# Hi-PACE/hipace

Measured on AMD Instinct MI355X. Metric: transverse slices/s at 1024^2 x 4ppc (explicit solver), higher is better.
Workload: dtype f64

## Files before the change

### hipace_amd/api.py

```python
import ctypes as C

import numpy as np
import torch

from . import _lib
from ._lib import CIDX, COMPS, ID_VALID, PL_REAL, check


def _stream():
    return C.c_void_p(torch.cuda.current_stream().cuda_stream)


def _iarr(vals):
    return (C.c_int * len(vals))(*[int(v) for v in vals])


class Geometry:

    def __init__(self, nx, ny, lo, hi, dz, bc=1, normalized=True, consts=(1., 1., 1., 1., 1.), ng=None):
        self.nx, self.ny = nx, ny
        g = _lib.Geom()
        g.dx = (hi[0] - lo[0]) / nx
        g.dy = (hi[1] - lo[1]) / ny
        g.dz = dz
        g.xoff = 0.5 * (lo[0] + hi[0] - g.dx * (nx - 1))
        g.yoff = 0.5 * (lo[1] + hi[1] - g.dy * (ny - 1))
        g.c, g.ep0, g.mu0, g.q_e, g.m_e = consts
        g.plo = (C.c_double * 2)(lo[0], lo[1])
        g.phi = (C.c_double * 2)(hi[0], hi[1])
        g.bc = bc
        g.normalized = int(normalized)
        self.c = g


class Fields:

    def __init__(self, nx, ny, ng, ncomp, device="cuda", data=None):
        self.nx, self.ny, self.ng, self.ncomp = nx, ny, ng, ncomp
        shape = (ncomp, ny + 2 * ng, nx + 2 * ng)
        if data is None:
            self.t = torch.zeros(shape, dtype=torch.float64, device=device)
        else:
            self.t = torch.as_tensor(np.ascontiguousarray(data), dtype=torch.float64).reshape(shape).to(device).contiguous()

    def struct(self):
        s = _lib.Slab()
        s.p = self.t.data_ptr()
        s.nx, s.ny, s.ng, s.ncomp = self.nx, self.ny, self.ng, self.ncomp
        s.jstride = self.nx + 2 * self.ng
        s.nstride = s.jstride * (self.ny + 2 * self.ng)
        return s

    def numpy(self):
        return self.t.cpu().numpy()


class PlasmaSheet:

    def __init__(self, real, valid=None, ion_lev=None, device="cuda", key=None):
        real = np.ascontiguousarray(real, dtype=np.float64)
        assert real.shape[0] == 11
        self.n = real.shape[1]
        self.real = torch.as_tensor(real).to(device).contiguous()
        if valid is None:
            valid = np.ones(self.n, dtype=np.int32)
        idcpu = np.where(np.asarray(valid) != 0, np.uint64(ID_VALID | (1 << 24)), np.uint64(1 << 24)).astype(np.uint64)
        if key is not None:
            ids = (np.asarray(key, dtype=np.uint64) + np.uint64(1)) << np.uint64(24)
            idcpu = (idcpu & np.uint64(ID_VALID)) | ids
        self.idcpu = torch.as_tensor(idcpu.view(np.int64)).to(device).contiguous()
        if ion_lev is None:
            ion_lev = np.zeros(self.n, dtype=np.int32)
        self.ion_lev = torch.as_tensor(np.asarray(ion_lev, dtype=np.int32)).to(device).contiguous()

    def struct(self):
        p = _lib.Plasma()
        base = self.real.data_ptr()
        for k, name in enumerate(PL_REAL):
            setattr(p, name, base + 8 * k * self.n)
        p.idcpu = self.idcpu.data_ptr()
        p.ion_lev = self.ion_lev.data_ptr()
        p.n = self.n
        return p

    def numpy(self):
        idc = self.idcpu.cpu().numpy().view(np.uint64)
        return self.real.cpu().numpy(), ((idc >> np.uint64(63)) & np.uint64(1)).astype(np.int32)


class BoxSorter:

    def sortParticlesByBox(self, z, plo_z, dz, num_boxes):
        z = z.contiguous()
        n = z.numel()
        counts = torch.zeros(num_boxes + 1, dtype=torch.int64, device=z.device)
        offsets = torch.zeros(num_boxes + 1, dtype=torch.int64, device=z.device)
        perm = torch.zeros(max(n, 1), dtype=torch.int64, device=z.device)
        check(_lib.lib().hps_beam_sort_by_box(C.c_void_p(z.data_ptr() if n else 0), n, float(plo_z), float(dz), num_boxes,
                                              C.c_void_p(counts.data_ptr()), C.c_void_p(offsets.data_ptr()),
                                              C.c_void_p(perm.data_ptr()), _stream()))
        torch.cuda.synchronize()
        self.boxCounts = counts.cpu().numpy().astype(np.uint64)
        self.boxOffsets = offsets.cpu().numpy().astype(np.uint64)
        self.boxPermutations = perm[:n].cpu().numpy().astype(np.uint64)
        return self


class Tiling:

    def __init__(self, nx, ny, tile_size, max_particles):
        self._h = C.c_void_p()
        check(_lib.lib().hps_tiling_create(nx, ny, tile_size, max_particles, C.byref(self._h)))
        self.fallback = torch.zeros(1, dtype=torch.int32, device="cuda")

    def reorder(self, plasma, geom):
        out = PlasmaSheet.__new__(PlasmaSheet)
        out.n = plasma.n
        out.real = torch.empty_like(plasma.real)
        out.idcpu = torch.empty_like(plasma.idcpu)
        out.ion_lev = torch.empty_like(plasma.ion_lev)
        check(_lib.lib().hps_reorder_particles(self._h, plasma.struct(), out.struct(), geom.c, _stream()))
        return out

    def set_validity(self, by_weight=False, by_psi_half=False):
        check(_lib.lib().hps_tiling_set_validity(self._h, int(by_weight), int(by_psi_half)))

    def info(self):
        nt, off, perm = C.c_int(), C.c_void_p(), C.c_void_p()
        check(_lib.lib().hps_tiling_info(self._h, C.byref(nt), C.byref(off), C.byref(perm)))
        return nt.value, off.value, perm.value

    def offsets_and_perm(self, n):
        torch.cuda.synchronize()
        nt, off, perm = self.info()
        o = np.empty(nt + 2, dtype=np.int32)
        p = np.empty(n, dtype=np.uint32)
        check(_lib.lib().hps_memcpy_d2h(o.ctypes.data_as(C.c_void_p), C.c_void_p(off), o.nbytes))
        if n:
            check(_lib.lib().hps_memcpy_d2h(p.ctypes.data_as(C.c_void_p), C.c_void_p(perm), p.nbytes))
        return o, p

    def __del__(self):
        if getattr(self, "_h", None) and _lib is not None:
            _lib.lib().hps_tiling_destroy(self._h)
            self._h = None


def DepositCurrent(plasma, fields, geom, charge, mass, depos_order, jx=-1, jy=-1, jz=-1, rho=-1, chi=-1,
                   rhomjz=-1, max_qsa_weighting_factor=35.0, can_ionize=False, n_qsa=None, tiling=None, aabs=-1):
    comp = _iarr([jx, jy, jz, rho, chi, rhomjz])
    nq = C.c_void_p(n_qsa.data_ptr()) if n_qsa is not None else None
    if tiling is None:
        check(_lib.lib().hps_deposit_current_laser(fields.struct(), plasma.struct(), geom.c, comp, aabs, charge, mass,
                                                   depos_order, max_qsa_weighting_factor, int(can_ionize), nq, _stream()))
    else:
        check(_lib.lib().hps_deposit_current_tiled_laser(fields.struct(), plasma.struct(), geom.c, comp, aabs, charge, mass,
                                                         depos_order, max_qsa_weighting_factor, int(can_ionize), nq,
                                                         tiling._h, C.c_void_p(tiling.fallback.data_ptr()), _stream()))


def ExplicitDeposition(plasma, fields, geom, charge, mass, depos_order, Bz, Ez, ExmBy, EypBx, Sy, Sx,
                       derivative_type=2, can_ionize=False, tiling=None, aabs=-1):
    if tiling is None:
        check(_lib.lib().hps_explicit_deposit_laser(fields.struct(), plasma.struct(), geom.c, _iarr([Bz, Ez, ExmBy, EypBx]),
                                                    aabs, _iarr([Sy, Sx]), charge, mass, depos_order, derivative_type,
                                                    int(can_ionize), _stream()))
    else:
        check(_lib.lib().hps_explicit_deposit_tiled_laser(fields.struct(), plasma.struct(), geom.c,
                                                          _iarr([Bz, Ez, ExmBy, EypBx]), aabs, _iarr([Sy, Sx]), charge, mass,
                                                          depos_order, derivative_type, int(can_ionize), tiling._h,
                                                          C.c_void_p(tiling.fallback.data_ptr()), _stream()))


def AdvancePlasmaParticles(plasma, fields, geom, charge, mass, depos_order, Psi, Ez, Bx, By, Bz,
                           temp_slice=False, n_subcycles=1, can_ionize=False, tiling=None, aabs=-1):
    if tiling is None:
        check(_lib.lib().hps_advance_plasma_laser(fields.struct(), plasma.struct(), geom.c, _iarr([Psi, Ez, Bx, By, Bz]),
                                                  aabs, charge, mass, depos_order, int(temp_slice), n_subcycles,
                                                  int(can_ionize), _stream()))
    else:
        check(_lib.lib().hps_advance_plasma_tiled_laser(fields.struct(), plasma.struct(), geom.c,
                                                        _iarr([Psi, Ez, Bx, By, Bz]), aabs, charge, mass, depos_order,
                                                        int(temp_slice), n_subcycles, int(can_ionize), tiling._h,
                                                        C.c_void_p(tiling.fallback.data_ptr()), _stream()))


def CoulombCollision(plasma_a, plasma_b, geom, charge_a, mass_a, charge_b=None, mass_b=None, can_ionize_a=False,
                     can_ionize_b=False, coulomb_log=-1.0, background_density_SI=0.0, seed=0, collision=0, step=0, islice=0,
                     tiling_a=None, tiling_b=None):
    if plasma_b is plasma_a or charge_b is None:
        charge_b, mass_b, can_ionize_b = charge_a, mass_a, can_ionize_a
    pairs, over = C.c_long(), C.c_long()
    check(_lib.lib().hps_collide_plasma(plasma_a.struct(), tiling_a._h if tiling_a is not None else None,
                                        plasma_b.struct(), tiling_b._h if tiling_b is not None else None, geom.c, geom.nx, geom.ny,
                                        charge_a, mass_a, int(can_ionize_a), charge_b, mass_b, int(can_ionize_b), coulomb_log,
                                        background_density_SI, seed, collision, step, islice, C.byref(pairs), C.byref(over),
                                        _stream()))
    return pairs.value, over.value


class BeamSlice:

    def __init__(self, soa, nsub=None, device="cuda"):
        soa = np.ascontiguousarray(soa, dtype=np.float64)
        assert soa.ndim == 2 and soa.shape[0] == 7
        self.n = soa.shape[1]
        self.soa = torch.as_tensor(soa).to(device).contiguous()
        self.nsub = None if nsub is None else torch.as_tensor(np.ascontiguousarray(nsub, dtype=np.int32)).to(device).contiguous()
        assert self.nsub is None or self.nsub.numel() == self.n

    def struct(self):
        b = _lib.BeamSlice()
        base = self.soa.data_ptr()
        for k, name in enumerate(("x", "y", "z", "ux", "uy", "uz", "w")):
            setattr(b, name, base + 8 * k * self.n)
        b.nsub = self.nsub.data_ptr() if self.nsub is not None else None
        b.n = self.n
        return b

    def numpy(self):
        return self.soa.cpu().numpy()


def BeamPlasmaCollision(beam, plasma, geom, charge_beam, mass_beam, charge_plasma, mass_plasma, dt, can_ionize_plasma=False,
                        coulomb_log=-1.0, background_density_SI=0.0, seed=0, collision=0, step=0, islice=0):
    pairs, over = C.c_long(), C.c_long()
    check(_lib.lib().hps_collide_beam_plasma(beam.struct(), plasma.struct(), geom.c, geom.nx, geom.ny, charge_beam, mass_beam,
                                             charge_plasma, mass_plasma, int(can_ionize_plasma), coulomb_log, background_density_SI,
                                             seed, collision, step, islice, dt, C.byref(pairs), C.byref(over), _stream()))
    return pairs.value, over.value


def record_particle_dispatch(on=True):
    check(_lib.lib().hps_particles_record(int(on)))


def recorded_particle_dispatch():
    n = C.c_long()
    check(_lib.lib().hps_particles_recorded(None, 0, C.byref(n)))
    buf = C.create_string_buffer(n.value + 1)
    check(_lib.lib().hps_particles_recorded(buf, n.value + 1, C.byref(n)))
    return set(buf.value.decode().split())


class FFTPoissonSolver:

    def __init__(self, nx, ny, dx, dy, device="cuda"):
        self.nx, self.ny = nx, ny
        self._h = C.c_void_p()
        check(_lib.lib().hps_poisson_create(nx, ny, dx, dy, C.byref(self._h)))
        self.staging = torch.zeros((ny, nx), dtype=torch.float64, device=device)

    def StagingArea(self):
        return self.staging

    BACKENDS = ("own-sym", "own-pow2", "dense", "rocfft")

    def info(self):
        b, n, m = C.c_int(), C.c_int(), C.c_int()
        check(_lib.lib().hps_poisson_info(self._h, C.byref(b), C.byref(n), C.byref(m)))
        return self.BACKENDS[b.value], n.value, m.value

    def SolvePoissonEquation(self, lhs_fields, comp):
        check(_lib.lib().hps_poisson_solve(self._h, C.c_void_p(self.staging.data_ptr()), lhs_fields.struct(), comp,
                                           _stream()))

    def __del__(self):
        if getattr(self, "_h", None) and _lib is not None:
            _lib.lib().hps_poisson_destroy(self._h)
            self._h = None


class MultiGrid2:

    def __init__(self, nx, ny, dx, dy):
        self._h = C.c_void_p()
        check(_lib.lib().hps_mg2_create(nx, ny, dx, dy, C.byref(self._h)))

    def solve2(self, sol2, rhs2, acoef_real, acoef_imag, tol_rel=1e-4, tol_abs=0.0, nummaxiter=200):
        it = C.c_int()
        rn = C.c_double()
        for t in (sol2, rhs2, acoef_real, acoef_imag):
            assert t.is_cuda and t.is_contiguous() and t.dtype == torch.float64
        check(_lib.lib().hps_mg2_solve2(self._h, sol2.data_ptr(), rhs2.data_ptr(), acoef_real.data_ptr(), acoef_imag.data_ptr(),
                                        tol_rel, tol_abs, nummaxiter, C.byref(it), C.byref(rn), _stream()))
        return it.value, rn.value

    BOTTOMS = ("lower-v", "single-block", "per-sweep")
    TILES = ("single-block", "32x16", "64x32")

    def info(self):
        nl, top, b, t = C.c_int(), C.c_int(), C.c_int(), (C.c_int * 31)()
        check(_lib.lib().hps_mg2_info(self._h, C.byref(nl), C.byref(top), C.byref(b), t))
        return {"nlev": nl.value, "low_top": top.value, "bottom": self.BOTTOMS[b.value],
                "tiles": tuple(self.TILES[v] for v in t if v >= 0)}

    def __del__(self):
        if getattr(self, "_h", None) and _lib is not None:
            _lib.lib().hps_mg2_destroy(self._h)
            self._h = None


class MultiGrid:

    def __init__(self, nx, ny, dx, dy):
        self._h = C.c_void_p()
        check(_lib.lib().hps_mg_create(nx, ny, dx, dy, C.byref(self._h)))

    LOWV = ("v3", "v-cc", "v-nodal", "bottom")
    TILES = ("TileSmall", "TileBig", "TileSmall-pull", "TileMid-pull")

    def info(self):
        cc, nl, lb, kind, npyr, nres, pull1 = (C.c_int() for _ in range(7))
        lds, t = C.c_long(), (C.c_int * 31)()
        check(_lib.lib().hps_mg_info(self._h, C.byref(cc), C.byref(nl), C.byref(lb), C.byref(kind), C.byref(lds), t,
                                     C.byref(pull1), C.byref(npyr), C.byref(nres)))
        return {"cc": bool(cc.value), "nlev": nl.value, "lowv_begin": lb.value, "lowv": self.LOWV[kind.value],
                "lowv_lds": lds.value, "tiles": tuple(self.TILES[v] for v in t if v >= 0), "nodal_pull1": bool(pull1.value),
                "pyramid": npyr.value, "restricts": nres.value}

    def solve1(self, fields, sol_comp, rhs_comp, acoef_comp, tol_rel=1e-4, tol_abs=2.2250738585072014e-308,
               nummaxiter=200):
        it = C.c_int()
        rn = C.c_double()
        check(_lib.lib().hps_mg_solve1(self._h, fields.struct(), sol_comp, rhs_comp, acoef_comp, tol_rel, tol_abs,
                                       nummaxiter, C.byref(it), C.byref(rn), _stream()))
        return it.value, rn.value

    def solve1_fabs(self, sol, rhs, acoef, tol_rel=1e-4, tol_abs=2.2250738585072014e-308, nummaxiter=200):
        it = C.c_int()
        rn = C.c_double()
        check(_lib.lib().hps_mg_solve1_fabs(self._h, sol.struct(), rhs.struct(), acoef.struct(), tol_rel, tol_abs, nummaxiter,
                                            C.byref(it), C.byref(rn), _stream()))
        return it.value, rn.value

    def __del__(self):
        if getattr(self, "_h", None) and _lib is not None:
            _lib.lib().hps_mg_destroy(self._h)
            self._h = None


class AdaptiveTimeStep:

    def __init__(self, deck, density_profile=None):
        self.deck = dict(deck)
        self._dk = _lib.fill_struct(_lib.Deck(), deck)
        self._h = C.c_void_p()
        check(_lib.lib().hps_adaptive_create(C.byref(self._dk), C.byref(self._h)))
        if density_profile is not None:
            self.set_density_profile(*density_profile)

    @classmethod
    def for_engine(cls, engine):
        return cls(engine.deck, getattr(engine, "density_profile", None))

    def __del__(self):
        if getattr(self, "_h", None) and _lib is not None:
            _lib.lib().hps_adaptive_destroy(self._h)
            self._h = None

    def set_density_profile(self, r=(), fr=(), ct=(), ft=()):
        a = [np.ascontiguousarray(v, dtype=np.float64) for v in (r, fr, ct, ft)]
        assert len(a[0]) == len(a[1]) and len(a[2]) == len(a[3])
        p = [x.ctypes.data_as(C.c_void_p) if len(x) else None for x in a]
        check(_lib.lib().hps_adaptive_set_density_profile(self._h, len(a[0]), p[0], p[1], len(a[2]), p[2], p[3]))

    def initial_dt(self, uz_mean=None, uz_std=None, nstages=1):
        um = self.deck["beam_umean"][2] if uz_mean is None else uz_mean
        us = self.deck.get("beam_uz_std", 0.0) if uz_std is None else uz_std
        dt = C.c_double()
        check(_lib.lib().hps_adaptive_initial_dt(self._h, float(um), float(us), int(nstages), C.byref(dt)))
        return dt.value

    def CalculateFromDensity(self, t):
        dt = C.c_double()
        check(_lib.lib().hps_adaptive_before_step(self._h, float(t), C.byref(dt)))
        return dt.value

    def next_time(self):
        t = C.c_double()
        check(_lib.lib().hps_adaptive_next_time(self._h, C.byref(t)))
        return t.value

    def CalculateFromMinUz(self, moments, t, nstages=1):
        m = np.ascontiguousarray(moments, dtype=np.float64)
        assert m.shape == (4,)
        dt = C.c_double()
        check(_lib.lib().hps_adaptive_after_step(self._h, m.ctypes.data_as(C.c_void_p), float(t), int(nstages), C.byref(dt)))
        return dt.value


class SliceEngine:

    def __init__(self, deck, device=0, tile_size=None, sort_period=None):
        self.deck = dict(deck)
        self.step_times = []
        self._dk = _lib.fill_struct(_lib.Deck(), deck)
        self._h = C.c_void_p()
        check(_lib.lib().hps_engine_create(C.byref(self._dk), device, C.byref(self._h)))
        if tile_size is not None:
            check(_lib.lib().hps_engine_set_tiling(self._h, tile_size, sort_period or 128))
        for a, b, coulomb_log, seed in deck.get("collisions", ()):
            if a == "beam":
                self.add_beam_collision(b, coulomb_log, seed)
            else:
                self.add_collision(a, b, coulomb_log, seed)
        nc, ng, npart = C.c_int(), C.c_int(), C.c_long()
        check(_lib.lib().hps_engine_info(self._h, C.byref(nc), C.byref(ng), C.byref(npart)))
        self.ncomp, self.ng, self.nparticles = nc.value, ng.value, npart.value

    def __del__(self):
        if getattr(self, "_h", None) and _lib is not None:
            _lib.lib().hps_engine_destroy(self._h)
            self._h = None

    def begin_step(self):
        check(_lib.lib().hps_engine_begin_step(self._h))

    def solve_slice(self, islice):
        check(_lib.lib().hps_engine_solve_slice(self._h, islice))

    def solve_slice_begin(self, islice):
        check(_lib.lib().hps_engine_solve_slice_begin(self._h, islice))

    def solve_slice_finish(self, islice):
        check(_lib.lib().hps_engine_solve_slice_finish(self._h, islice))

    def slice_ready(self):
        return bool(_lib.lib().hps_engine_slice_ready(self._h))

    def run_step(self):
        check(_lib.lib().hps_engine_run_step(self._h))

    def sync(self):
        check(_lib.lib().hps_engine_sync(self._h))

    def set_tiling(self, tile_size=16, sort_period=128):
        check(_lib.lib().hps_engine_set_tiling(self._h, tile_size, sort_period))

    def add_collision(self, species_a=0, species_b=0, coulomb_log=-1.0, seed=0):
        check(_lib.lib().hps_engine_add_collision(self._h, species_a, species_b, coulomb_log, seed))

    def add_beam_collision(self, plasma_species=0, coulomb_log=-1.0, seed=0):
        check(_lib.lib().hps_engine_add_beam_collision(self._h, plasma_species, coulomb_log, seed))

    def collision_stats(self):
        a, b = C.c_long(), C.c_long()
        check(_lib.lib().hps_engine_collision_stats(self._h, C.byref(a), C.byref(b)))
        return dict(pairs_collided=a.value, overfull_cells=b.value)

    @property
    def moving(self):
        return float(self.deck.get("dt", 0.0)) != 0.0 or self.adaptive

    @property
    def adaptive(self):
        return bool(self.deck.get("dt_adaptive", 0))

    def set_time(self, t, dt):
        check(_lib.lib().hps_engine_set_time(self._h, float(t), float(dt)))

    def beam_moments(self):
        out = np.zeros(4, dtype=np.float64)
        check(_lib.lib().hps_engine_beam_moments(self._h, out.ctypes.data_as(C.c_void_p)))
        return out

    def run_adaptive(self, n_steps=None, controller=None, on_step_end=None):
        assert self.adaptive, "run_adaptive needs a deck with dt_adaptive"
        n = self.deck["n_steps"] if n_steps is None else int(n_steps)
        ats = controller or AdaptiveTimeStep.for_engine(self)
        ats.initial_dt(nstages=1)
        t, log = 0.0, []
        for step in range(n):
            if t == float("inf"):
                break
            dt = ats.CalculateFromDensity(t)
            log.append((step, t, dt))
            self.set_time(t, dt)
            self.run_step()
            ats.CalculateFromMinUz(self.beam_moments(), t, 1)
            if on_step_end is not None:
                on_step_end(step, t, dt)
            t = ats.next_time()
        return log

    def beam_capacity(self):
        n = C.c_long()
        check(_lib.lib().hps_engine_beam_capacity(self._h, C.byref(n)))
        return n.value

    def set_beam_capacity(self, cap):
        check(_lib.lib().hps_engine_set_beam_capacity(self._h, int(cap)))

    def beam_message_doubles(self):
        r = C.c_int()
        check(_lib.lib().hps_engine_beam_message_rows(self._h, C.byref(r)))
        return 1 + r.value * self.beam_capacity()

    def beam_spin(self):
        nbeam, _ = self.beam_layout()
        out = np.zeros((3, max(nbeam, 1)), dtype=np.float64)
        check(_lib.lib().hps_engine_beam_spin(self._h, out.ctypes.data_as(C.c_void_p) if nbeam else None))
        return out[:, :nbeam]

    def set_beam_import(self, on):
        check(_lib.lib().hps_engine_set_beam_import(self._h, int(on)))

    def export_beam_slice(self, islice, msg):
        check(_lib.lib().hps_engine_export_beam_slice(self._h, islice, C.c_void_p(msg.data_ptr())))

    def import_beam_slice(self, islice, msg):
        check(_lib.lib().hps_engine_import_beam_slice(self._h, islice, C.c_void_p(msg.data_ptr())))

    def beam_state(self):
        nbeam, _ = self.beam_layout()
        nz = self.deck["nz"]
        bnd = np.zeros(nz + 1, dtype=np.int64)
        soa = np.zeros((7, max(nbeam, 1)), dtype=np.float64)
        check(_lib.lib().hps_engine_beam_state(self._h, bnd.ctypes.data_as(C.c_void_p), soa.ctypes.data_as(C.c_void_p) if nbeam else None))
        return bnd, soa[:, :nbeam].reshape(7, nbeam) if nbeam else soa[:, :0]

    def set_density_profile(self, r=(), fr=(), ct=(), ft=()):
        self.density_profile = (r, fr, ct, ft)
        a = [np.ascontiguousarray(v, dtype=np.float64) for v in (r, fr, ct, ft)]
        assert len(a[0]) == len(a[1]) and len(a[2]) == len(a[3])
        p = [x.ctypes.data_as(C.c_void_p) if len(x) else None for x in a]
        check(_lib.lib().hps_engine_set_density_profile(self._h, len(a[0]), p[0], p[1], len(a[2]), p[2], p[3]))

    def set_fusion(self, on=True):
        check(_lib.lib().hps_engine_set_fusion(self._h, int(on)))

    def fallbacks(self):
        n = C.c_long()
        check(_lib.lib().hps_engine_fallbacks(self._h, C.byref(n)))
        return n.value

    def sorts(self):
        n = C.c_long()
        check(_lib.lib().hps_engine_sorts(self._h, C.byref(n)))
        return n.value

    def set_diagnostics(self, on=True):
        check(_lib.lib().hps_engine_set_diagnostics(self._h, int(on)))

    def set_profiling(self, on=True, stride=1, light=False):
        check(_lib.lib().hps_engine_set_profiling_stride(self._h, int(stride)))
        check(_lib.lib().hps_engine_set_profiling(self._h, (2 if light else 1) if on else 0))

    def beam_layout(self):
        nb = C.c_long()
        off = (C.c_long * (self.deck["nz"] + 1))()
        check(_lib.lib().hps_engine_beam_info(self._h, C.byref(nb), off))
        return nb.value, np.array(off[:], dtype=np.int64)

    def set_beam_particles(self, soa, allow_outside=False):
        soa = np.ascontiguousarray(soa, dtype=np.float64)
        assert soa.ndim == 2 and soa.shape[0] == 7
        out = C.c_long(0)
        check(_lib.lib().hps_engine_set_beam_particles(self._h, soa.shape[1], soa.ctypes.data_as(C.c_void_p),
                                                       C.byref(out) if allow_outside else None))
        return out.value

    def set_beam_storage(self, tensor, injected_beam_support=False):
        check(_lib.lib().hps_engine_set_beam_storage(self._h, C.c_void_p(tensor.data_ptr()) if tensor is not None else None))
        if tensor is not None and injected_beam_support:
            check(_lib.lib().hps_engine_assume_initial_beam_support(self._h))

    def initial_beam_into(self, tensor):
        check(_lib.lib().hps_engine_initial_beam(self._h, C.c_void_p(tensor.data_ptr())))

    def set_field_diagnostic(self, names, coarsening=(1, 1, 1), diag_type="xyz", patch_lo=None, patch_hi=None):
        idx = _lib.CIDX_PC if self.deck.get("bxby_solver", 0) else _lib.CIDX
        cn = self.comp_names()
        comps = (C.c_int * len(names))(*[idx[n] if n in idx else cn.index(n) for n in names])
        co = (C.c_int * 3)(*coarsening)
        sd = {"xyz": -1, "yz": 0, "xz": 1, "xy": 2}[diag_type]
        plo = (C.c_double * 3)(*patch_lo) if patch_lo is not None else None
        phi = (C.c_double * 3)(*patch_hi) if patch_hi is not None else None
        check(_lib.lib().hps_engine_set_field_diagnostic_box(self._h, len(names), comps, co, sd, plo, phi))
        self._fd = (list(names), tuple(coarsening))

    def field_diagnostic_geometry(self):
        n, lo, hi = (C.c_int * 3)(), (C.c_double * 3)(), (C.c_double * 3)()
        check(_lib.lib().hps_engine_field_diagnostic_geometry(self._h, n, lo, hi))
        return tuple(n), tuple(lo), tuple(hi)

    def field_diagnostic(self):
        names, _ = self._fd
        n, _, _ = self.field_diagnostic_geometry()
        out = np.empty((len(names), n[2], n[1], n[0]))
        check(_lib.lib().hps_engine_field_diagnostic(self._h, out.ctypes.data_as(C.c_void_p)))
        return {k: out[i] for i, k in enumerate(names)}

    INSITU_FIELDS = ["[Ex^2]", "[Ey^2]", "[Ez^2]", "[Bx^2]", "[By^2]", "[Bz^2]", "[ExmBy^2]", "[EypBx^2]", "[jz_beam]",
                     "[Ez*jz_beam]"]

    INSITU_PLASMA = ["sum(w)", "[x]", "[x^2]", "[y]", "[y^2]", "[ux]", "[ux^2]", "[uy]", "[uy^2]", "[uz]", "[uz^2]", "[ga]",
                     "[ga^2]", "[(ga-1)*(1-vz)]", "Np"]

    INSITU_BEAM = ["sum(w)", "[x]", "[x^2]", "[y]", "[y^2]", "[z]", "[z^2]", "[ux]", "[ux^2]", "[uy]", "[uy^2]", "[uz]", "[uz^2]",
                   "[x*ux]", "[y*uy]", "[z*uz]", "[x*uy]", "[y*ux]", "[ux/uz]", "[uy/uz]", "[ga]", "[ga^2]", "Np"]

    def laser_vcycles(self):
        n = C.c_long()
        check(_lib.lib().hps_engine_laser_vcycles(self._h, C.byref(n)))
        return n.value

    def set_insitu_beam(self, radius=float("inf")):
        check(_lib.lib().hps_engine_set_insitu_beam(self._h, min(float(radius), 1.0e300)))

    def insitu_beam(self):
        out = np.empty((23, self.deck["nz"]))
        check(_lib.lib().hps_engine_insitu_beam(self._h, out.ctypes.data_as(C.c_void_p)))
        return {n: out[i] for i, n in enumerate(self.INSITU_BEAM)}

    def set_insitu_plasma(self, radius=float("inf")):
        check(_lib.lib().hps_engine_set_insitu_plasma(self._h, min(float(radius), 1.0e300)))

    def insitu_plasma(self):
        out = np.empty((15, self.deck["nz"]))
        check(_lib.lib().hps_engine_insitu_plasma(self._h, out.ctypes.data_as(C.c_void_p)))
        return {n: out[i] for i, n in enumerate(self.INSITU_PLASMA)}

    def set_insitu_fields(self, on=True):
        check(_lib.lib().hps_engine_set_insitu_fields(self._h, int(on)))

    def insitu_fields(self):
        out = np.empty((10, self.deck["nz"]))
        check(_lib.lib().hps_engine_insitu_fields(self._h, out.ctypes.data_as(C.c_void_p)))
        return {n: out[i] for i, n in enumerate(self.INSITU_FIELDS)}

    def stream_handle(self):
        return _lib.lib().hps_engine_stream(self._h)

    def record_event(self, slot):
        ev = C.c_void_p()
        check(_lib.lib().hps_engine_record_event(self._h, int(slot), C.byref(ev)))
        return ev.value

    def wait_event(self, event):
        if event is not None:
            check(_lib.lib().hps_engine_wait_event(self._h, C.c_void_p(event)))

    def copy_async(self, dst, src):
        assert dst.numel() == src.numel()
        check(_lib.lib().hps_engine_copy_async(self._h, C.c_void_p(dst.data_ptr()), C.c_void_p(src.data_ptr()),
                                               dst.numel() * 8))

    def phase_times(self):
        ms = (C.c_double * 8)()
        n = C.c_long()
        check(_lib.lib().hps_engine_phase_times(self._h, ms, C.byref(n)))
        names = ["deposit_current", "poisson", "explicit_deposit", "mg_solve1", "advance_plasma", "other", "sort", "empty_interval"]
        return {k: ms[i] for i, k in enumerate(names)}, n.value

    def checksums(self):
        out = (C.c_double * self.ncomp)()
        check(_lib.lib().hps_engine_checksums(self._h, out))
        names = self.comp_names()
        cs = {names[i]: out[i] for i in range(self.ncomp)}
        if "aabs" in cs:
            tot = C.c_double()
            check(_lib.lib().hps_engine_laser_info(self._h, None, C.byref(tot)))
            cs["laserEnvelope"] = tot.value
        return cs

    @property
    def has_laser(self):
        return bool(self.deck.get("laser_on", 0))

    def laser_message_doubles(self):
        return 4 * self.deck["nx"] * self.deck["ny"]

    def set_step(self, step):
        check(_lib.lib().hps_engine_set_step(self._h, int(step)))

    def set_laser_import(self, on, step=0):
        check(_lib.lib().hps_engine_set_laser_import(self._h, int(on), int(step)))

    def export_laser_slice(self, islice, msg):
        check(_lib.lib().hps_engine_export_laser_slice(self._h, islice, C.c_void_p(msg.data_ptr())))

    def import_laser_slice(self, islice, msg):
        check(_lib.lib().hps_engine_import_laser_slice(self._h, islice, C.c_void_p(msg.data_ptr())))

    def import_laser_from(self, islice, src):
        check(_lib.lib().hps_engine_import_laser_from(self._h, islice, src._h))

    def laser_envelope(self):
        d = self.deck
        out = np.empty((d["nz"], d["ny"], d["nx"]), dtype=np.complex128)
        check(_lib.lib().hps_engine_laser_envelope(self._h, out.ctypes.data_as(C.c_void_p)))
        return out

    def comp_names(self):
        if self.deck.get("bxby_solver", 0):
            return list(_lib.COMPS_PC[:22]) + (["rho"] if self.deck.get("deposit_rho", 0) else [])
        return list(COMPS[:21]) + (["rho"] if self.deck.get("deposit_rho", 0) else []) + \
            (["aabs"] if self.deck.get("laser_on", 0) else []) + \
            (["Salame_" + n for n in _lib.COMPS_SALAME] if self.deck.get("beam_do_salame", 0) else [])

    def salame_stats(self):
        nz = self.deck["nz"]
        out = np.zeros((nz, 4), dtype=np.float64)
        check(_lib.lib().hps_engine_salame_stats(self._h, out.ctypes.data_as(C.c_void_p)))
        flags = out[:, 3].astype(np.int64)
        return {"W": out[:, 0].copy(), "W_total": out[:, 1].copy(), "iterations": out[:, 2].astype(np.int64),
                "converged": (flags & 1) != 0, "overloaded": (flags & 2) != 0, "ran": out[:, 2] > 0}

    def pc_stats(self):
        its, err = C.c_long(), C.c_double()
        check(_lib.lib().hps_engine_pc_stats(self._h, C.byref(its), C.byref(err)))
        return its.value, err.value

    def pc_zero_b_slices(self):
        n = C.c_long()
        check(_lib.lib().hps_engine_pc_zero_b_slices(self._h, C.byref(n)))
        return n.value

    def stats(self):
        vc, sl = C.c_long(), C.c_long()
        check(_lib.lib().hps_engine_stats(self._h, C.byref(vc), C.byref(sl)))
        return dict(vcycles=vc.value, slices=sl.value)

    def slab(self):
        self.sync()
        s = _lib.lib().hps_engine_slab(self._h)
        nx, ny, g = s.nx, s.ny, s.ng
        out = np.empty((s.ncomp, ny + 2 * g, nx + 2 * g), dtype=np.float64)
        check(_lib.lib().hps_memcpy_d2h(out.ctypes.data_as(C.c_void_p), C.c_void_p(s.p), out.nbytes))
        return out

    def ions(self):
        self.sync()
        p = _lib.lib().hps_engine_ions(self._h)
        n = p.n
        real = np.empty((11, n), dtype=np.float64)
        idc = np.empty(n, dtype=np.uint64)
        lev = np.empty(n, dtype=np.int32)
        if n:
            for k, name in enumerate(PL_REAL):
                check(_lib.lib().hps_memcpy_d2h(real[k].ctypes.data_as(C.c_void_p), C.c_void_p(getattr(p, name)), real[k].nbytes))
            check(_lib.lib().hps_memcpy_d2h(idc.ctypes.data_as(C.c_void_p), C.c_void_p(p.idcpu), idc.nbytes))
            check(_lib.lib().hps_memcpy_d2h(lev.ctypes.data_as(C.c_void_p), C.c_void_p(p.ion_lev), lev.nbytes))
        key = ((idc >> np.uint64(24)) & np.uint64((1 << 39) - 1)).astype(np.int64) - 1
        return real, ((idc >> np.uint64(63)) & np.uint64(1)).astype(np.int32), lev, key

    def ion_stats(self):
        a, b = C.c_long(), C.c_long()
        check(_lib.lib().hps_engine_ion_stats(self._h, C.byref(a), C.byref(b)))
        return a.value, b.value

    def particles(self):
        self.sync()
        p = _lib.lib().hps_engine_plasma(self._h)
        n = p.n
        real = np.empty((11, n), dtype=np.float64)
        idc = np.empty(n, dtype=np.uint64)
        if n:
            for k, name in enumerate(PL_REAL):
                check(_lib.lib().hps_memcpy_d2h(real[k].ctypes.data_as(C.c_void_p), C.c_void_p(getattr(p, name)), real[k].nbytes))
            check(_lib.lib().hps_memcpy_d2h(idc.ctypes.data_as(C.c_void_p), C.c_void_p(p.idcpu), idc.nbytes))
        return real, ((idc >> np.uint64(63)) & np.uint64(1)).astype(np.int32)
```

### hipace_amd/csrc/sort.hip

```cpp
#include "common.h"
#include "tiling.h"

#include <cstdlib>
#include <cstring>
#include <rocprim/device/device_radix_sort.hpp>

namespace hps {

constexpr int RANK_CAP = 16;

__host__ __device__ __forceinline__ int cell_in_tile (int x, int y, int ts, int bw)
{
    if (bw >= ts) return y*ts + x;
    const int bh = 32/bw;
    const int bx = x/bw, by = y/bh, nbx = ts/bw;
    return ((by*nbx + bx)*bh + (y - by*bh))*bw + (x - bx*bw);
}

__device__ __forceinline__ unsigned int cell_key (double x, double y, uint64_t id, const TileGeom& t)
{
    const int ncell = t.ts*t.ts;
    if (!(id & HPS_ID_VALID)) return (unsigned int)(t.ntiles*ncell);
    int ci = (int)floor((x - t.xoff)*t.dx_inv + 0.5);
    int cj = (int)floor((y - t.yoff)*t.dy_inv + 0.5);
    ci = min(max(ci, 0), t.nx - 1);
    cj = min(max(cj, 0), t.ny - 1);
    const int tile = (cj / t.ts)*t.ntx + (ci / t.ts);
    return (unsigned int)(tile*ncell + cell_in_tile(ci % t.ts, cj % t.ts, t.ts, t.bw));
}

__global__ __launch_bounds__(256)
void k_cell_keys (hps_plasma pl, TileGeom t, unsigned int* keys, unsigned int* idx)
{
    const long p = (long)blockIdx.x*blockDim.x + threadIdx.x;
    if (p >= pl.n) return;
    keys[p] = cell_key(pl.x[p], pl.y[p], pl.idcpu[p], t);
    idx[p] = (unsigned int)p;
}

__global__ __launch_bounds__(256)
void k_run_starts (const unsigned int* keys, long n, int nkeys, int* first)
{
    const long p = (long)blockIdx.x*blockDim.x + threadIdx.x;
    if (p > n) return;
    const int prev = (p == 0) ? -1 : (int)keys[p - 1];
    const int cur = (p == n) ? nkeys : (int)keys[p];
    for (int k = prev + 1; k <= cur; ++k) first[k] = (int)p;
}

__global__ __launch_bounds__(256)
void k_rank_keys (const unsigned int* ckeys, const int* first, long n, int ncell, unsigned int* keys2)
{
    const long p = (long)blockIdx.x*blockDim.x + threadIdx.x;
    if (p >= n) return;
    const unsigned int ck = ckeys[p];
    const int rank = min((int)p - first[ck], RANK_CAP - 1);
    const unsigned int tile = ck / ncell, cit = ck - tile*ncell;
    keys2[p] = (tile*RANK_CAP + rank)*ncell + cit;
}

__global__ __launch_bounds__(256)
void k_tile_offsets (const unsigned int* keys, long n, int ntiles, int per_tile, int* offsets)
{
    const long p = (long)blockIdx.x*blockDim.x + threadIdx.x;
    if (p > n) return;
    const int prev = (p == 0) ? -1 : (int)(keys[p - 1]/per_tile);
    const int cur = (p == n) ? ntiles + 1 : (int)(keys[p]/per_tile);
    for (int t = prev + 1; t <= cur; ++t) offsets[t] = (int)p;
}

__global__ __launch_bounds__(256)
void k_tile_order_keys (const int* offsets, int ntiles, unsigned int* keys, unsigned int* vals)
{
    const int t = blockIdx.x*blockDim.x + threadIdx.x;
    if (t >= ntiles) return;
    keys[t] = 0xFFFFFFFFu - (unsigned int)(offsets[t + 1] - offsets[t]);
    vals[t] = (unsigned int)t;
}
__global__ __launch_bounds__(256)
void k_tile_order_identity (int* order, int ntiles)
{
    const int t = blockIdx.x*blockDim.x + threadIdx.x;
    if (t < ntiles) order[t] = t;
}
__global__ __launch_bounds__(256)
void k_tile_launch_info (const int* offsets, int ntiles, int4* launch)
{
    const int b = blockIdx.x*blockDim.x + threadIdx.x;
    if (b >= ntiles) return;
    const int t = offsets[ntiles + 2 + b];
    launch[b] = make_int4(t, offsets[t], offsets[t + 1], 0);
}

__global__ __launch_bounds__(256)
void k_permute (hps_plasma src, hps_plasma dst, const unsigned int* perm)
{
    const long p = (long)blockIdx.x*blockDim.x + threadIdx.x;
    if (p >= src.n) return;
    const unsigned int q = perm[p];
    dst.x[p] = src.x[q]; dst.y[p] = src.y[q]; dst.w[p] = src.w[q];
    dst.ux[p] = src.ux[q]; dst.uy[p] = src.uy[q]; dst.psi[p] = src.psi[q];
    if (dst.x_prev != dst.x) dst.x_prev[p] = src.x_prev[q];
    if (dst.y_prev != dst.y) dst.y_prev[p] = src.y_prev[q];
    dst.ux_half[p] = src.ux_half[q]; dst.uy_half[p] = src.uy_half[q]; dst.psi_half[p] = src.psi_half[q];
    dst.idcpu[p] = src.idcpu[q]; dst.ion_lev[p] = src.ion_lev[q];
}

Tiling::~Tiling ()
{
    (void)hipFree(offsets); (void)hipFree(keys_a); (void)hipFree(keys_b); (void)hipFree(idx_a); (void)hipFree(idx_b);
    (void)hipFree(temp); (void)hipFree(cell_first); (void)hipFree(okeys); (void)hipFree(otemp);
}

int tiling_create (int nx, int ny, int ts, long capacity, Tiling** out)
{
    if (ts != 16 && ts != 32) { set_error("hps_tiling_create: tile_size must be 16 or 32"); return HPS_ERR_ARG; }
    Tiling* T = new Tiling;
    T->g.nx = nx; T->g.ny = ny; T->g.ts = ts;
    T->g.ntx = (nx + ts - 1)/ts; T->g.nty = (ny + ts - 1)/ts; T->g.ntiles = T->g.ntx*T->g.nty;
    T->g.bw = 32;
    if (const char* e = std::getenv("HPS_CELL_BLOCK_W")) { const int v = std::atoi(e); if (v == 4 || v == 8 || v == 16 || v == 32) T->g.bw = v; }
    if (T->g.bw > ts) T->g.bw = ts;
    T->capacity = capacity;
    HPS_HIP_CHECK(hipMalloc(&T->offsets, (tile_launch_offset(T->g.ntiles) + 4*T->g.ntiles)*sizeof(int)));
    HPS_HIP_CHECK(hipMemset(T->offsets, 0, (tile_launch_offset(T->g.ntiles) + 4*T->g.ntiles)*sizeof(int)));
    hipLaunchKernelGGL(k_tile_order_identity, dim3(ceil_div(T->g.ntiles, 256)), dim3(256), 0, (hipStream_t)0, T->offsets + T->g.ntiles + 2, T->g.ntiles);
    hipLaunchKernelGGL(k_tile_launch_info, dim3(ceil_div(T->g.ntiles, 256)), dim3(256), 0, (hipStream_t)0, T->offsets, T->g.ntiles, reinterpret_cast<int4*>(T->offsets + tile_launch_offset(T->g.ntiles)));
    HPS_HIP_CHECK(hipDeviceSynchronize());
    HPS_HIP_CHECK(hipMalloc(&T->okeys, 3*(size_t)T->g.ntiles*sizeof(unsigned int)));
    HPS_HIP_CHECK(rocprim::radix_sort_pairs(nullptr, T->otemp_bytes, T->okeys, T->okeys, T->okeys, T->okeys, (size_t)T->g.ntiles, 0, 32, (hipStream_t)0));
    HPS_HIP_CHECK(hipMalloc(&T->otemp, T->otemp_bytes));
    HPS_HIP_CHECK(hipMalloc(&T->keys_a, capacity*sizeof(unsigned int)));
    HPS_HIP_CHECK(hipMalloc(&T->keys_b, capacity*sizeof(unsigned int)));
    HPS_HIP_CHECK(hipMalloc(&T->idx_a, capacity*sizeof(unsigned int)));
    HPS_HIP_CHECK(hipMalloc(&T->idx_b, capacity*sizeof(unsigned int)));
    const long ncell = (long)ts*ts;
    const long nkeys1 = (long)T->g.ntiles*ncell + 1;
    const long nkeys2 = ((long)T->g.ntiles*RANK_CAP + 1)*ncell;
    if (nkeys2 >= (1L << 31)) { delete T; set_error("hps_tiling_create: grid too large for 32-bit sort keys"); return HPS_ERR_ARG; }
    int bits = 1; while ((1L << bits) < nkeys1) ++bits;
    T->key_bits = bits;
    bits = 1; while ((1L << bits) < nkeys2) ++bits;
    T->key2_bits = bits;
    HPS_HIP_CHECK(hipMalloc(&T->cell_first, (nkeys1 + 1)*sizeof(int)));
    HPS_HIP_CHECK(rocprim::radix_sort_pairs(nullptr, T->temp_bytes, T->keys_a, T->keys_b, T->idx_a, T->idx_b,
                                            (size_t)capacity, 0, T->key2_bits, (hipStream_t)0));
    HPS_HIP_CHECK(hipMalloc(&T->temp, T->temp_bytes));
    *out = T;
    return HPS_OK;
}

int tiling_sort (Tiling* T, const hps_plasma& src, const hps_plasma& dst, const hps_geom& g, hipStream_t st)
{
    if (src.n > T->capacity) { set_error("hps_reorder_particles: more particles than the tiling capacity"); return HPS_ERR_ARG; }
    T->g.xoff = g.xoff; T->g.yoff = g.yoff; T->g.dx_inv = 1.0/g.dx; T->g.dy_inv = 1.0/g.dy;
    const long n = src.n;
    if (n == 0) {
        HPS_HIP_CHECK(hipMemsetAsync(T->offsets, 0, (T->g.ntiles + 2)*sizeof(int), st));
        hipLaunchKernelGGL(k_tile_launch_info, dim3(ceil_div(T->g.ntiles, 256)), dim3(256), 0, st, T->offsets, T->g.ntiles, reinterpret_cast<int4*>(T->offsets + tile_launch_offset(T->g.ntiles)));
        T->sorted_n = 0; return HPS_OK;
    }
    const int ncell = T->g.ts*T->g.ts;
    const int nkeys1 = T->g.ntiles*ncell + 1;
    const dim3 gn(ceil_div(n, 256)), gn1(ceil_div(n + 1, 256)), b256(256);
    hipLaunchKernelGGL(k_cell_keys, gn, b256, 0, st, src, T->g, T->keys_a, T->idx_a);
    size_t tb = T->temp_bytes;
    HPS_HIP_CHECK(rocprim::radix_sort_pairs(T->temp, tb, T->keys_a, T->keys_b, T->idx_a, T->idx_b, (size_t)n, 0,
                                            T->key_bits, st));
    hipLaunchKernelGGL(k_run_starts, gn1, b256, 0, st, T->keys_b, n, nkeys1, T->cell_first);
    hipLaunchKernelGGL(k_rank_keys, gn, b256, 0, st, T->keys_b, T->cell_first, n, ncell, T->keys_a);
    tb = T->temp_bytes;
    HPS_HIP_CHECK(rocprim::radix_sort_pairs(T->temp, tb, T->keys_a, T->keys_b, T->idx_b, T->idx_a, (size_t)n, 0,
                                            T->key2_bits, st));
    hipLaunchKernelGGL(k_tile_offsets, gn1, b256, 0, st, T->keys_b, n, T->g.ntiles, RANK_CAP*ncell, T->offsets);
    hipLaunchKernelGGL(k_permute, dim3(ceil_div(n, 256)), dim3(256), 0, st, src, dst, T->idx_a);
    {   const int nt = T->g.ntiles;
        unsigned int *ka = T->okeys, *kb = T->okeys + nt, *va = T->okeys + 2*nt;
        hipLaunchKernelGGL(k_tile_order_keys, dim3(ceil_div(nt, 256)), b256, 0, st, T->offsets, nt, ka, va);
        size_t ob = T->otemp_bytes;
        HPS_HIP_CHECK(rocprim::radix_sort_pairs(T->otemp, ob, ka, kb, va, reinterpret_cast<unsigned int*>(T->offsets + nt + 2), (size_t)nt, 0, 32, st));
        hipLaunchKernelGGL(k_tile_launch_info, dim3(ceil_div(nt, 256)), b256, 0, st, T->offsets, nt, reinterpret_cast<int4*>(T->offsets + tile_launch_offset(nt))); }
    HPS_HIP_CHECK(hipGetLastError());
    T->sorted_n = n;
    return HPS_OK;
}

__global__ __launch_bounds__(256)
void k_box_keys (const double* __restrict__ z, long n, double plo_z, double dzi, int num_boxes, unsigned int* keys, unsigned int* idx)
{
    const long i = (long)blockIdx.x*blockDim.x + threadIdx.x;
    if (i >= n) return;
    int b = static_cast<int>((z[i] - plo_z)*dzi);
    if (b < 0 || b > num_boxes) b = num_boxes;
    keys[i] = (unsigned int)b; idx[i] = (unsigned int)i;
}

__global__ __launch_bounds__(256)
void k_box_offsets (const unsigned int* keys, long n, int num_boxes, unsigned long long* counts, unsigned long long* offsets)
{
    const long p = (long)blockIdx.x*blockDim.x + threadIdx.x;
    if (p > n) return;
    const int prev = (p == 0) ? -1 : (int)keys[p - 1];
    const int cur = (p == n) ? num_boxes + 1 : (int)keys[p];
    for (int k = prev + 1; k <= cur && k <= num_boxes; ++k) offsets[k] = (unsigned long long)p;
    (void)counts;
}
__global__ __launch_bounds__(256)
void k_box_counts (long n, int num_boxes, const unsigned int* idx, unsigned long long* counts, const unsigned long long* offsets,
                   unsigned long long* perm)
{
    const long p = (long)blockIdx.x*blockDim.x + threadIdx.x;
    if (p < n) perm[p] = idx[p];
    if (p <= num_boxes) counts[p] = (p == num_boxes ? (unsigned long long)n : offsets[p + 1]) - offsets[p];
}

}

using namespace hps;

extern "C" int hps_beam_sort_by_box (const double* z_dev, long n, double plo_z, double dz, int num_boxes,
                                     unsigned long long* counts_dev, unsigned long long* offsets_dev,
                                     unsigned long long* perm_dev, hps_stream stream)
{
    HPS_REQUIRE(n >= 0 && num_boxes >= 1 && counts_dev && offsets_dev && (perm_dev || n == 0) && (z_dev || n == 0),
                "hps_beam_sort_by_box: bad argument");
    HPS_REQUIRE(n < (1L << 32), "hps_beam_sort_by_box: more than 2^32 particles");
    hipStream_t st = (hipStream_t)stream;
    const size_t nb1 = (size_t)num_boxes + 1;
    if (n == 0) {
        HPS_HIP_CHECK(hipMemsetAsync(counts_dev, 0, nb1*sizeof(unsigned long long), st));
        HPS_HIP_CHECK(hipMemsetAsync(offsets_dev, 0, nb1*sizeof(unsigned long long), st));
        return HPS_OK;
    }
    unsigned int *ka = nullptr, *kb = nullptr, *ia = nullptr, *ib = nullptr; void* temp = nullptr; size_t tb = 0;
    int bits = 1; while ((1L << bits) < (long)nb1) ++bits;
    HPS_HIP_CHECK(hipMalloc(&ka, 4*(size_t)n*sizeof(unsigned int)));
    kb = ka + n; ia = kb + n; ib = ia + n;
    HPS_HIP_CHECK(rocprim::radix_sort_pairs(nullptr, tb, ka, kb, ia, ib, (size_t)n, 0, bits, st));
    HPS_HIP_CHECK(hipMalloc(&temp, tb));
    const dim3 b256(256);
    hipLaunchKernelGGL(k_box_keys, dim3(ceil_div(n, 256)), b256, 0, st, z_dev, n, plo_z, 1.0/dz, num_boxes, ka, ia);
    HPS_HIP_CHECK(rocprim::radix_sort_pairs(temp, tb, ka, kb, ia, ib, (size_t)n, 0, bits, st));
    const long span = std::max<long>(n + 1, (long)nb1);
    hipLaunchKernelGGL(k_box_offsets, dim3(ceil_div(n + 1, 256)), b256, 0, st, kb, n, num_boxes, counts_dev, offsets_dev);
    hipLaunchKernelGGL(k_box_counts, dim3(ceil_div(span, 256)), b256, 0, st, n, num_boxes, ib, counts_dev, offsets_dev, perm_dev);
    HPS_HIP_CHECK(hipGetLastError());
    HPS_HIP_CHECK(hipStreamSynchronize(st));
    (void)hipFree(ka); (void)hipFree(temp);
    return HPS_OK;
}

extern "C" int hps_tiling_create (int nx, int ny, int tile_size, long max_particles, void** handle)
{
    HPS_REQUIRE(nx > 0 && ny > 0 && max_particles >= 0 && handle, "hps_tiling_create: bad argument");
    HPS_REQUIRE(max_particles < (1L << 28), "hps_tiling_create: at most 2^28 particles per tile-sorted sheet (32-bit offsets in the tile kernels)");
    Tiling* T = nullptr;
    if (int e = tiling_create(nx, ny, tile_size, std::max(max_particles, 1L), &T)) return e;
    *handle = T;
    return HPS_OK;
}

extern "C" int hps_reorder_particles (void* tiling, hps_plasma src, hps_plasma dst, hps_geom geom, hps_stream stream)
{
    HPS_REQUIRE(tiling, "hps_reorder_particles: null tiling");
    HPS_REQUIRE(dst.n >= src.n || src.n == 0, "hps_reorder_particles: destination too small");
    return tiling_sort(static_cast<Tiling*>(tiling), src, dst, geom, (hipStream_t)stream);
}

extern "C" int hps_tiling_info (void* tiling, int* ntiles, const int** offsets_dev, const unsigned int** perm_dev)
{
    Tiling* T = static_cast<Tiling*>(tiling);
    if (ntiles) *ntiles = T->g.ntiles;
    if (offsets_dev) *offsets_dev = T->offsets;
    if (perm_dev) *perm_dev = T->idx_a;
    return HPS_OK;
}

extern "C" int hps_tiling_destroy (void* tiling) { delete static_cast<Tiling*>(tiling); return HPS_OK; }

extern "C" int hps_tiling_set_validity (void* tiling, int by_weight, int by_psi_half)
{
    if (!tiling) { set_error("hps_tiling_set_validity: null tiling"); return HPS_ERR_ARG; }
    Tiling* T = static_cast<Tiling*>(tiling);
    T->valid_by_w = by_weight != 0;
    T->valid_by_psi = by_psi_half != 0;
    return HPS_OK;
}
```

### hipace_amd/csrc/tiling.h

```cpp
#ifndef HPS_TILING_H_
#define HPS_TILING_H_
#include "common.h"

namespace hps {

struct TileGeom { int nx, ny, ts, ntx, nty, ntiles; double xoff, yoff, dx_inv, dy_inv;
                  int bw;
};

struct Tiling {
    TileGeom g{};
    long capacity = 0, sorted_n = 0;
    int* offsets = nullptr;
    unsigned int *okeys = nullptr; void* otemp = nullptr; size_t otemp_bytes = 0;
    unsigned int *keys_a = nullptr, *keys_b = nullptr, *idx_a = nullptr, *idx_b = nullptr;
    void* temp = nullptr; size_t temp_bytes = 0; int key_bits = 0, key2_bits = 0;
    int* cell_first = nullptr;
    bool valid_by_psi = false;
    bool valid_by_w = false;
    ~Tiling ();
};

struct TailWork { int first = 0, nwg = 0; const unsigned long long* live_n = nullptr;
                  int extra = 0; };

__host__ __device__ inline int tile_launch_offset (int ntiles) { return (2*ntiles + 2 + 3) & ~3; }

int tiling_create (int nx, int ny, int ts, long capacity, Tiling** out);
int tiling_sort (Tiling* T, const hps_plasma& src, const hps_plasma& dst, const hps_geom& g, hipStream_t st);

}
#endif
```

Baseline: 1666.

## Replace second radix sort with per-tile rank placement and rank-count tile ordering

The second radix sort over (tile, rank, cell) keys is replaced by a per-tile kernel. It computes each particle's interleaved position from the cell run starts using ballots and a shared-memory scan, then writes the permutation directly. The radix sort that orders tiles by particle count is replaced, for up to 8192 tiles, by a single kernel that counts ranks in shared memory. This removes a full-size sort pass plus two helper kernels from every slice's sort, at the cost of more complex kernels whose load depends on per-tile imbalance. A Python helper for reading back the launch order is also added.

```diff
diff --git a/hipace_amd/api.py b/hipace_amd/api.py
--- a/hipace_amd/api.py
+++ b/hipace_amd/api.py
@@ -139,6 +139,15 @@
         if n:
             check(_lib.lib().hps_memcpy_d2h(p.ctypes.data_as(C.c_void_p), C.c_void_p(perm), p.nbytes))
         return o, p
+
+    def launch_order(self):
+        torch.cuda.synchronize()
+        nt, off, _ = self.info()
+        order = np.empty(nt, dtype=np.int32)
+        rec = np.empty((nt, 4), dtype=np.int32)
+        check(_lib.lib().hps_memcpy_d2h(order.ctypes.data_as(C.c_void_p), C.c_void_p(off + 4 * (nt + 2)), order.nbytes))
+        check(_lib.lib().hps_memcpy_d2h(rec.ctypes.data_as(C.c_void_p), C.c_void_p(off + 4 * ((2 * nt + 2 + 3) & ~3)), rec.nbytes))
+        return order, rec
 
     def __del__(self):
         if getattr(self, "_h", None) and _lib is not None:
diff --git a/hipace_amd/csrc/sort.hip b/hipace_amd/csrc/sort.hip
--- a/hipace_amd/csrc/sort.hip
+++ b/hipace_amd/csrc/sort.hip
@@ -48,25 +48,67 @@
     for (int k = prev + 1; k <= cur; ++k) first[k] = (int)p;
 }
 
-__global__ __launch_bounds__(256)
-void k_rank_keys (const unsigned int* ckeys, const int* first, long n, int ncell, unsigned int* keys2)
-{
-    const long p = (long)blockIdx.x*blockDim.x + threadIdx.x;
-    if (p >= n) return;
-    const unsigned int ck = ckeys[p];
-    const int rank = min((int)p - first[ck], RANK_CAP - 1);
-    const unsigned int tile = ck / ncell, cit = ck - tile*ncell;
-    keys2[p] = (tile*RANK_CAP + rank)*ncell + cit;
-}
-
-__global__ __launch_bounds__(256)
-void k_tile_offsets (const unsigned int* keys, long n, int ntiles, int per_tile, int* offsets)
-{
-    const long p = (long)blockIdx.x*blockDim.x + threadIdx.x;
-    if (p > n) return;
-    const int prev = (p == 0) ? -1 : (int)(keys[p - 1]/per_tile);
-    const int cur = (p == n) ? ntiles + 1 : (int)(keys[p]/per_tile);
-    for (int t = prev + 1; t <= cur; ++t) offsets[t] = (int)p;
+template <int K>
+__global__ __launch_bounds__(256)
+void k_tile_place (const int* __restrict__ cell_first, const unsigned int* __restrict__ idx_sorted, int ntiles, int n,
+                   unsigned int* __restrict__ perm, int* __restrict__ offsets)
+{
+    constexpr int NW = 4, NE = RANK_CAP*K*NW, PER = NE/64, CAP = RANK_CAP - 1;
+    __shared__ int base[NE];
+    const int t = blockIdx.x, tid = threadIdx.x, lane = tid & 63, w = tid >> 6;
+    const int c0 = t*(K*256);
+    int first[K], cnt[K], capx[K];
+#pragma unroll
+    for (int k = 0; k < K; ++k) {
+        const int c = c0 + k*256 + tid;
+        first[k] = cell_first[c];
+        cnt[k] = cell_first[c + 1] - first[k];
+    }
+#pragma unroll
+    for (int k = 0; k < K; ++k) {
+#pragma unroll
+        for (int r = 0; r < CAP; ++r) {
+            const unsigned long long b = __ballot(cnt[k] > r);
+            if (lane == 0) base[(r*K + k)*NW + w] = __popcll(b);
+        }
+        const int over = max(cnt[k] - CAP, 0);
+        int incl = over;
+#pragma unroll
+        for (int d = 1; d < 64; d <<= 1) { const int v = __shfl_up(incl, d); if (lane >= d) incl += v; }
+        capx[k] = incl - over;
+        if (lane == 63) base[(CAP*K + k)*NW + w] = incl;
+    }
+    __syncthreads();
+    if (w == 0) {
+        int v[PER], s = 0;
+#pragma unroll
+        for (int j = 0; j < PER; ++j) { v[j] = base[lane*PER + j]; s += v[j]; }
+        int incl = s;
+#pragma unroll
+        for (int d = 1; d < 64; d <<= 1) { const int u = __shfl_up(incl, d); if (lane >= d) incl += u; }
+        int run = incl - s;
+#pragma unroll
+        for (int j = 0; j < PER; ++j) { base[lane*PER + j] = run; run += v[j]; }
+    }
+    __syncthreads();
+    const int tfirst = cell_first[c0];
+    const unsigned long long below = (1ull << lane) - 1ull;
+#pragma unroll
+    for (int k = 0; k < K; ++k) {
+        for (int r = 0; r < CAP; ++r) {
+            const unsigned long long b = __ballot(cnt[k] > r);
+            if (b == 0) break;
+            if (cnt[k] > r) perm[tfirst + base[(r*K + k)*NW + w] + __popcll(b & below)] = idx_sorted[first[k] + r];
+        }
+        const int place = tfirst + base[(CAP*K + k)*NW + w] + capx[k];
+        for (int r = CAP; r < cnt[k]; ++r) perm[place + r - CAP] = idx_sorted[first[k] + r];
+    }
+    const int inv0 = cell_first[ntiles*(K*256)];
+    if (tid == 0) {
+        offsets[t] = tfirst;
+        if (t == 0) { offsets[ntiles] = inv0; offsets[ntiles + 1] = n; }
+    }
+    for (long p = (long)inv0 + (long)t*256 + tid; p < n; p += (long)gridDim.x*256) perm[p] = idx_sorted[p];
 }
 
 __global__ __launch_bounds__(256)
@@ -90,6 +132,48 @@
     if (b >= ntiles) return;
     const int t = offsets[ntiles + 2 + b];
     launch[b] = make_int4(t, offsets[t], offsets[t + 1], 0);
+}
+
+constexpr int ORDER_TILES = 16, ORDER_PARTS = 64, ORDER_THREADS = ORDER_TILES*ORDER_PARTS, ORDER_COUNT_MAX = 8192;
+__global__ __launch_bounds__(ORDER_THREADS)
+void k_tile_launch_order (int* offsets, int ntiles, int4* launch)
+{
+    constexpr int NPAD = ORDER_COUNT_MAX + 4*ORDER_PARTS, PER = NPAD/ORDER_THREADS + 1;
+    __shared__ __attribute__((aligned(16))) int cnt[NPAD];
+    __shared__ int part[ORDER_THREADS/64][ORDER_TILES];
+    const int tid = threadIdx.x;
+    const int len = ((ntiles + ORDER_PARTS - 1)/ORDER_PARTS + 3) & ~3;
+    int first[PER], end[PER];
+#pragma unroll
+    for (int k = 0; k < PER; ++k) {
+        const int i = min(tid + k*ORDER_THREADS, ntiles - 1);
+        first[k] = offsets[i]; end[k] = offsets[i + 1];
+    }
+#pragma unroll
+    for (int k = 0; k < PER; ++k) {
+        const int i = tid + k*ORDER_THREADS;
+        if (i < len*ORDER_PARTS) cnt[i] = i < ntiles ? end[k] - first[k] : -1;
+    }
+    __syncthreads();
+    const int j = tid & (ORDER_TILES - 1), q = tid/ORDER_TILES;
+    const int t = blockIdx.x*ORDER_TILES + j;
+    const int c = cnt[min(t, ntiles - 1)];
+    int pos = 0;
+    for (int u = q*len; u < (q + 1)*len; u += 4) {
+        const int4 v = *reinterpret_cast<const int4*>(&cnt[u]);
+        pos += (v.x > c - (u < t)) + (v.y > c - (u + 1 < t)) + (v.z > c - (u + 2 < t)) + (v.w > c - (u + 3 < t));
+    }
+#pragma unroll
+    for (int d = ORDER_TILES; d < 64; d <<= 1) pos += __shfl_xor(pos, d);
+    if ((tid & 63) < ORDER_TILES) part[tid >> 6][j] = pos;
+    __syncthreads();
+    if (tid < ORDER_TILES && t < ntiles) {
+        int p = 0;
+#pragma unroll
+        for (int k = 0; k < ORDER_THREADS/64; ++k) p += part[k][tid];
+        offsets[ntiles + 2 + p] = t;
+        launch[p] = make_int4(t, offsets[t], offsets[t + 1], 0);
+    }
 }
 
 __global__ __launch_bounds__(256)
@@ -127,24 +211,23 @@
     hipLaunchKernelGGL(k_tile_order_identity, dim3(ceil_div(T->g.ntiles, 256)), dim3(256), 0, (hipStream_t)0, T->offsets + T->g.ntiles + 2, T->g.ntiles);
     hipLaunchKernelGGL(k_tile_launch_info, dim3(ceil_div(T->g.ntiles, 256)), dim3(256), 0, (hipStream_t)0, T->offsets, T->g.ntiles, reinterpret_cast<int4*>(T->offsets + tile_launch_offset(T->g.ntiles)));
     HPS_HIP_CHECK(hipDeviceSynchronize());
-    HPS_HIP_CHECK(hipMalloc(&T->okeys, 3*(size_t)T->g.ntiles*sizeof(unsigned int)));
-    HPS_HIP_CHECK(rocprim::radix_sort_pairs(nullptr, T->otemp_bytes, T->okeys, T->okeys, T->okeys, T->okeys, (size_t)T->g.ntiles, 0, 32, (hipStream_t)0));
-    HPS_HIP_CHECK(hipMalloc(&T->otemp, T->otemp_bytes));
+    if (T->g.ntiles > ORDER_COUNT_MAX) {
+        HPS_HIP_CHECK(hipMalloc(&T->okeys, 3*(size_t)T->g.ntiles*sizeof(unsigned int)));
+        HPS_HIP_CHECK(rocprim::radix_sort_pairs(nullptr, T->otemp_bytes, T->okeys, T->okeys, T->okeys, T->okeys, (size_t)T->g.ntiles, 0, 32, (hipStream_t)0));
+        HPS_HIP_CHECK(hipMalloc(&T->otemp, T->otemp_bytes));
+    }
     HPS_HIP_CHECK(hipMalloc(&T->keys_a, capacity*sizeof(unsigned int)));
     HPS_HIP_CHECK(hipMalloc(&T->keys_b, capacity*sizeof(unsigned int)));
     HPS_HIP_CHECK(hipMalloc(&T->idx_a, capacity*sizeof(unsigned int)));
     HPS_HIP_CHECK(hipMalloc(&T->idx_b, capacity*sizeof(unsigned int)));
     const long ncell = (long)ts*ts;
     const long nkeys1 = (long)T->g.ntiles*ncell + 1;
-    const long nkeys2 = ((long)T->g.ntiles*RANK_CAP + 1)*ncell;
-    if (nkeys2 >= (1L << 31)) { delete T; set_error("hps_tiling_create: grid too large for 32-bit sort keys"); return HPS_ERR_ARG; }
+    if (nkeys1 >= (1L << 31)) { delete T; set_error("hps_tiling_create: grid too large for 32-bit sort keys"); return HPS_ERR_ARG; }
     int bits = 1; while ((1L << bits) < nkeys1) ++bits;
     T->key_bits = bits;
-    bits = 1; while ((1L << bits) < nkeys2) ++bits;
-    T->key2_bits = bits;
     HPS_HIP_CHECK(hipMalloc(&T->cell_first, (nkeys1 + 1)*sizeof(int)));
     HPS_HIP_CHECK(rocprim::radix_sort_pairs(nullptr, T->temp_bytes, T->keys_a, T->keys_b, T->idx_a, T->idx_b,
-                                            (size_t)capacity, 0, T->key2_bits, (hipStream_t)0));
+                                            (size_t)capacity, 0, T->key_bits, (hipStream_t)0));
     HPS_HIP_CHECK(hipMalloc(&T->temp, T->temp_bytes));
     *out = T;
     return HPS_OK;
@@ -168,18 +251,19 @@
     HPS_HIP_CHECK(rocprim::radix_sort_pairs(T->temp, tb, T->keys_a, T->keys_b, T->idx_a, T->idx_b, (size_t)n, 0,
                                             T->key_bits, st));
     hipLaunchKernelGGL(k_run_starts, gn1, b256, 0, st, T->keys_b, n, nkeys1, T->cell_first);
-    hipLaunchKernelGGL(k_rank_keys, gn, b256, 0, st, T->keys_b, T->cell_first, n, ncell, T->keys_a);
-    tb = T->temp_bytes;
-    HPS_HIP_CHECK(rocprim::radix_sort_pairs(T->temp, tb, T->keys_a, T->keys_b, T->idx_b, T->idx_a, (size_t)n, 0,
-                                            T->key2_bits, st));
-    hipLaunchKernelGGL(k_tile_offsets, gn1, b256, 0, st, T->keys_b, n, T->g.ntiles, RANK_CAP*ncell, T->offsets);
+    if (ncell == 256) hipLaunchKernelGGL(k_tile_place<1>, dim3(T->g.ntiles), b256, 0, st, T->cell_first, T->idx_b, T->g.ntiles, (int)n, T->idx_a, T->offsets);
+    else hipLaunchKernelGGL(k_tile_place<4>, dim3(T->g.ntiles), b256, 0, st, T->cell_first, T->idx_b, T->g.ntiles, (int)n, T->idx_a, T->offsets);
     hipLaunchKernelGGL(k_permute, dim3(ceil_div(n, 256)), dim3(256), 0, st, src, dst, T->idx_a);
-    {   const int nt = T->g.ntiles;
+    const int nt = T->g.ntiles;
+    int4* launch = reinterpret_cast<int4*>(T->offsets + tile_launch_offset(nt));
+    if (nt <= ORDER_COUNT_MAX)
+        hipLaunchKernelGGL(k_tile_launch_order, dim3(ceil_div(nt, ORDER_TILES)), dim3(ORDER_THREADS), 0, st, T->offsets, nt, launch);
+    else {
         unsigned int *ka = T->okeys, *kb = T->okeys + nt, *va = T->okeys + 2*nt;
         hipLaunchKernelGGL(k_tile_order_keys, dim3(ceil_div(nt, 256)), b256, 0, st, T->offsets, nt, ka, va);
         size_t ob = T->otemp_bytes;
         HPS_HIP_CHECK(rocprim::radix_sort_pairs(T->otemp, ob, ka, kb, va, reinterpret_cast<unsigned int*>(T->offsets + nt + 2), (size_t)nt, 0, 32, st));
-        hipLaunchKernelGGL(k_tile_launch_info, dim3(ceil_div(nt, 256)), b256, 0, st, T->offsets, nt, reinterpret_cast<int4*>(T->offsets + tile_launch_offset(nt))); }
+        hipLaunchKernelGGL(k_tile_launch_info, dim3(ceil_div(nt, 256)), b256, 0, st, T->offsets, nt, launch); }
     HPS_HIP_CHECK(hipGetLastError());
     T->sorted_n = n;
     return HPS_OK;
diff --git a/hipace_amd/csrc/tiling.h b/hipace_amd/csrc/tiling.h
--- a/hipace_amd/csrc/tiling.h
+++ b/hipace_amd/csrc/tiling.h
@@ -14,7 +14,7 @@
     int* offsets = nullptr;
     unsigned int *okeys = nullptr; void* otemp = nullptr; size_t otemp_bytes = 0;
     unsigned int *keys_a = nullptr, *keys_b = nullptr, *idx_a = nullptr, *idx_b = nullptr;
-    void* temp = nullptr; size_t temp_bytes = 0; int key_bits = 0, key2_bits = 0;
+    void* temp = nullptr; size_t temp_bytes = 0; int key_bits = 0;
     int* cell_first = nullptr;
     bool valid_by_psi = false;
     bool valid_by_w = false;
```

Result: faster. 1689, median of 6 (+1.4%).
